# aicodix/modem

Measured on AMD Instinct MI355X. Metric: decoded frames/sec + BER, mode-6 8kHz OFDM, batch 65536, 1/2/4/8 MI355X, higher is better.
Workload: dtype f32

## Files before the change

modem_amd/csrc/k_theilsen.hip:

```cpp
#include "dev_common.h"
#include "kernels.h"

namespace rx {

#define TS_CAP 56
#define TS_OPEN_NEED 30
#define TS_OPEN_MARGIN 6
#define TS_MARGIN 12
#define TS_UNC_STEPS 24
constexpr int TS_QBITS = 22;
constexpr uint32_t TS_QREAL = (1u << TS_QBITS) - 8192u;
constexpr uint32_t TS_QPAD0 = (1u << TS_QBITS) - 4096u;
constexpr uint32_t TS_MQ = 2;
constexpr int TS_MQ1S = (int)((TS_MQ + 1) << 9);
constexpr int TS_LIST = 64;
constexpr int TS_MAX_IT = 48;
constexpr uint32_t TS_SENTINEL = 0x7fffffffu;

constexpr int TS_YS = 68, TS_PS = 76;
#define TS_ROWS_PER_WG 1
#define TS_SYNC() __syncthreads()
struct TsLds {
	float y[8 * TS_YS];
	uint2 sk[8 * TS_PS];
	uint32_t lst[TS_LIST];
};
__device__ __forceinline__ int ts_yaddr(int i) { return (i & 7) * TS_YS + (i >> 3); }
__device__ __forceinline__ int ts_paddr(int p) { return (p & 7) * TS_PS + (p >> 3); }

__device__ __forceinline__ unsigned fkey(float v)
{
	unsigned b = __float_as_uint(v);
	return (b & 0x80000000u) ? ~b : (b | 0x80000000u);
}
__device__ __forceinline__ float fkey_inv(unsigned k)
{
	unsigned b = (k & 0x80000000u) ? (k & 0x7fffffffu) : ~k;
	return __uint_as_float(b);
}
__device__ __forceinline__ float sub_mul_nofma(float y, float s, float x)
{
	#pragma clang fp contract(off)
	float p = s * x;
	return y - p;
}

__device__ __forceinline__ uint32_t med3u(uint32_t a, uint32_t b, uint32_t c)
{
	uint32_t r;
	asm("v_med3_u32 %0, %1, %2, %3" : "=v"(r) : "v"(a), "v"(b), "v"(c));
	return r;
}
template <int CTRL> __device__ __forceinline__ uint32_t dpp_u(uint32_t v)
{
	return (uint32_t)__builtin_amdgcn_mov_dpp((int)v, CTRL, 0xf, 0xf, true);
}
template <int PAT> __device__ __forceinline__ uint32_t swz_u(uint32_t v)
{
	return (uint32_t)__builtin_amdgcn_ds_swizzle((int)v, PAT);
}
constexpr int DPP_XOR1 = 0xB1, DPP_XOR2 = 0x4E, DPP_XOR3 = 0x1B, DPP_HALF_MIRROR = 0x141, DPP_MIRROR = 0x140, DPP_ROR8 = 0x128;
constexpr int SWZ_XOR4 = 0x101F, SWZ_XOR16 = 0x401F, SWZ_XOR31 = 0x7C1F;

struct TsLane {
	uint32_t c1, c2, c4, c8, c16, c32;
	int a63;
	int lane;
};
__device__ __forceinline__ TsLane ts_lane(int lane)
{
	TsLane L;
	L.c1 = (lane & 1) ? ~0u : 0u; L.c2 = (lane & 2) ? ~0u : 0u; L.c4 = (lane & 4) ? ~0u : 0u;
	L.c8 = (lane & 8) ? ~0u : 0u; L.c16 = (lane & 16) ? ~0u : 0u; L.c32 = (lane & 32) ? ~0u : 0u;
	L.a63 = (lane ^ 63) << 2;
	L.lane = lane;
	return L;
}
__device__ __forceinline__ int wave_sum_i(int v)
{
	v += (int)dpp_u<DPP_XOR1>((uint32_t)v);
	v += (int)dpp_u<DPP_XOR2>((uint32_t)v);
	v += (int)dpp_u<DPP_HALF_MIRROR>((uint32_t)v);
	v += (int)dpp_u<DPP_MIRROR>((uint32_t)v);
	return __builtin_amdgcn_readlane(v, 0) + __builtin_amdgcn_readlane(v, 16) + __builtin_amdgcn_readlane(v, 32) + __builtin_amdgcn_readlane(v, 48);
}
__device__ __forceinline__ float ts_uni(float v) { return __uint_as_float(__builtin_amdgcn_readfirstlane(__float_as_uint(v))); }
template <typename Op> __device__ __forceinline__ float wave_reduce_f(float v, Op op)
{
	v = op(v, __uint_as_float(dpp_u<DPP_XOR1>(__float_as_uint(v))));
	v = op(v, __uint_as_float(dpp_u<DPP_XOR2>(__float_as_uint(v))));
	v = op(v, __uint_as_float(dpp_u<DPP_HALF_MIRROR>(__float_as_uint(v))));
	v = op(v, __uint_as_float(dpp_u<DPP_MIRROR>(__float_as_uint(v))));
	const float a = __uint_as_float(__builtin_amdgcn_readlane(__float_as_uint(v), 0)), b = __uint_as_float(__builtin_amdgcn_readlane(__float_as_uint(v), 16));
	const float c = __uint_as_float(__builtin_amdgcn_readlane(__float_as_uint(v), 32)), d = __uint_as_float(__builtin_amdgcn_readlane(__float_as_uint(v), 48));
	return ts_uni(op(op(a, b), op(c, d)));
}

__device__ __forceinline__ void ts_ce(uint32_t &a, uint32_t &b)
{
	const uint32_t lo = a < b ? a : b, hi = a < b ? b : a;
	a = lo; b = hi;
}
template <int D> __device__ __forceinline__ void ts_stage(uint32_t (&k)[8], const TsLane &L)
{
	uint32_t p[8];
	#pragma unroll
	for (int t = 0; t < 8; ++t) {
		if (D == 1) p[t] = dpp_u<DPP_XOR1>(k[t]);
		else if (D == 2) p[t] = dpp_u<DPP_XOR2>(k[t]);
		else if (D == 4) p[t] = swz_u<SWZ_XOR4>(k[t]);
		else if (D == 8) p[t] = dpp_u<DPP_ROR8>(k[t]);
		else p[t] = swz_u<SWZ_XOR16>(k[t]);
	}
	__builtin_amdgcn_sched_barrier(0);
	const uint32_t c = D == 1 ? L.c1 : D == 2 ? L.c2 : D == 4 ? L.c4 : D == 8 ? L.c8 : L.c16;
	#pragma unroll
	for (int t = 0; t < 8; ++t)
		k[t] = med3u(k[t], p[t], c);
	__builtin_amdgcn_sched_barrier(0);
}
template <int M> __device__ __forceinline__ void ts_level(uint32_t (&k)[8], const TsLane &L)
{
	uint32_t p[8];
	#pragma unroll
	for (int t = 0; t < 8; ++t) {
		if (M == 1) p[t] = dpp_u<DPP_XOR1>(k[7 - t]);
		else if (M == 2) p[t] = dpp_u<DPP_XOR3>(k[7 - t]);
		else if (M == 3) p[t] = dpp_u<DPP_HALF_MIRROR>(k[7 - t]);
		else if (M == 4) p[t] = dpp_u<DPP_MIRROR>(k[7 - t]);
		else if (M == 5) p[t] = swz_u<SWZ_XOR31>(k[7 - t]);
		else p[t] = (uint32_t)__builtin_amdgcn_ds_bpermute(L.a63, (int)k[7 - t]);
	}
	__builtin_amdgcn_sched_barrier(0);
	{
		const uint32_t c = M == 1 ? L.c1 : M == 2 ? L.c2 : M == 3 ? L.c4 : M == 4 ? L.c8 : M == 5 ? L.c16 : L.c32;
		#pragma unroll
		for (int t = 0; t < 8; ++t)
			k[t] = med3u(k[t], p[t], c);
	}
	__builtin_amdgcn_sched_barrier(0);
	if (M >= 6) ts_stage<16>(k, L);
	if (M >= 5) ts_stage<8>(k, L);
	if (M >= 4) ts_stage<4>(k, L);
	if (M >= 3) ts_stage<2>(k, L);
	if (M >= 2) ts_stage<1>(k, L);
	ts_ce(k[0], k[4]); ts_ce(k[1], k[5]); ts_ce(k[2], k[6]); ts_ce(k[3], k[7]);
	ts_ce(k[0], k[2]); ts_ce(k[1], k[3]); ts_ce(k[4], k[6]); ts_ce(k[5], k[7]);
	ts_ce(k[0], k[1]); ts_ce(k[2], k[3]); ts_ce(k[4], k[5]); ts_ce(k[6], k[7]);
}
template <int M> __device__ __forceinline__ uint32_t ts_level_count(const uint32_t (&k)[8], const TsLane &L)
{
	uint32_t acc = 0;
	#pragma unroll
	for (int t = 0; t < 8; ++t)
		acc += ((k[t] >> (M + 2)) & 1u) * (256u + t);
	const uint32_t pbase = ((uint32_t)L.lane << 3) & ((16u << (M - 1)) - 1u);
	return (acc >> 8) * pbase + (acc & 255u);
}
constexpr int ts_inv_const()
{
	int c = 0;
	for (int m = 1; m <= 6; ++m) {
		const int k = 8 << m, l = k / 2, runs = 512 / k;
		c += runs * (k * (k - 1) / 2 - l * (l - 1) / 2);
	}
	return c;
}
constexpr int TS_INV_CONST = ts_inv_const();

__device__ __forceinline__ int ts_sort(uint32_t (&k)[8], const TsLane &L, bool counting, int levels)
{
	int share = 0;
	if (counting) {
		uint32_t h = 0;
		#pragma unroll
		for (int t = 0; t < 8; ++t)
			#pragma unroll
			for (int u = t + 1; u < 8; ++u)
				h = __builtin_amdgcn_alignbit(h, k[u] - k[t], 31);
		share = __popc(h);
	}
	ts_ce(k[0], k[1]); ts_ce(k[2], k[3]); ts_ce(k[4], k[5]); ts_ce(k[6], k[7]);
	ts_ce(k[0], k[2]); ts_ce(k[1], k[3]); ts_ce(k[4], k[6]); ts_ce(k[5], k[7]);
	ts_ce(k[1], k[2]); ts_ce(k[5], k[6]);
	ts_ce(k[0], k[4]); ts_ce(k[1], k[5]); ts_ce(k[2], k[6]); ts_ce(k[3], k[7]);
	ts_ce(k[2], k[4]); ts_ce(k[3], k[5]);
	ts_ce(k[1], k[2]); ts_ce(k[3], k[4]); ts_ce(k[5], k[6]);
	ts_level<1>(k, L); if (counting) share -= (int)ts_level_count<1>(k, L);
	ts_level<2>(k, L); if (counting) share -= (int)ts_level_count<2>(k, L);
	ts_level<3>(k, L); if (counting) share -= (int)ts_level_count<3>(k, L);
	ts_level<4>(k, L); if (counting) share -= (int)ts_level_count<4>(k, L);
	if (levels > 4) {
		ts_level<5>(k, L); if (counting) share -= (int)ts_level_count<5>(k, L);
		ts_level<6>(k, L); if (counting) share -= (int)ts_level_count<6>(k, L);
	}
	return share;
}

struct TsQuant { double scale, off; };
__device__ __forceinline__ TsQuant ts_quant(float T, float ymin, float ymax, int n)
{
	const double half = fabs((double)T) * (double)(n / 2 + 1);
	const double lo = (double)ymin - half, span = ((double)ymax + half) - lo;
	float sp = (float)span;
	sp = sp > 1e-30f ? sp : 1e-30f;
	const double scale = (double)(__builtin_amdgcn_rcpf(sp) * ((float)(TS_QREAL - 2u) * (1.f - 9.5367431640625e-7f)));
	TsQuant q;
	q.scale = scale;
	q.off = -lo * scale;
	return q;
}
__device__ __forceinline__ void ts_keys_run(uint32_t (&k)[8], const float (&yv)[8], int idx0, int n, float T, const TsQuant &q)
{
	const double tds = (double)T * q.scale;
	double c = fma(-tds, (double)(idx0 - n / 2), q.off);
	#pragma unroll
	for (int t = 0; t < 8; ++t) {
		const uint32_t qv = (uint32_t)fma((double)yv[t], q.scale, c);
		const int idx = idx0 + t;
		const uint32_t pad = TS_QPAD0 + 8u * (uint32_t)(idx - n + 1);
		k[t] = ((idx < n ? qv : pad) << 9) | (uint32_t)idx;
		c -= tds;
	}
}
__device__ __forceinline__ uint32_t ts_key(float y, int idx, int n, float T, const TsQuant &q)
{
	const double c = fma(-(double)T * q.scale, (double)(idx - n / 2), q.off);
	const uint32_t qv = (uint32_t)fma((double)y, q.scale, c);
	const uint32_t pad = TS_QPAD0 + 8u * (uint32_t)(idx - n + 1);
	return ((idx < n ? qv : pad) << 9) | (uint32_t)idx;
}

__device__ __forceinline__ float ts_pair_slope(const TsLds &s, int a, int b)
{
	const int i = a < b ? a : b, j = a < b ? b : a;
	return (s.y[ts_yaddr(j)] - s.y[ts_yaddr(i)]) / (float)(j - i);
}

__device__ __noinline__ float ts_slow_select(TsLds &s, int n, int lane, int target)
{
	uint32_t prefix = 0, mask = 0;
	int rank = target;
	uint32_t *hist = (uint32_t *)s.sk;
	for (int shift = 24; shift >= 0; shift -= 8) {
		for (int b = lane; b < 256; b += 64)
			hist[b] = 0;
		TS_SYNC();
		for (int d = 1; d < n; ++d) {
			const float fd = (float)d;
			for (int i = lane; i < n - d; i += 64) {
				const unsigned key = fkey((s.y[ts_yaddr(i + d)] - s.y[ts_yaddr(i)]) / fd);
				if ((key & mask) == prefix)
					atomicAdd(&hist[(key >> shift) & 255u], 1u);
			}
		}
		TS_SYNC();
		const uint32_t h0 = hist[4 * lane], h1 = hist[4 * lane + 1], h2 = hist[4 * lane + 2], h3 = hist[4 * lane + 3];
		const int mine = (int)(h0 + h1 + h2 + h3);
		int incl = mine;
		#pragma unroll
		for (int o = 1; o < 64; o <<= 1) {
			const int v = __shfl_up(incl, o);
			if (lane >= o)
				incl += v;
		}
		const int excl = incl - mine;
		const bool here = rank >= excl && rank < incl;
		int bin = 0, rr = 0;
		if (here) {
			rr = rank - excl;
			bin = 4 * lane;
			if (rr >= (int)h0) { rr -= h0; ++bin; if (rr >= (int)h1) { rr -= h1; ++bin; if (rr >= (int)h2) { rr -= h2; ++bin; } } }
		}
		const unsigned long long m = __builtin_amdgcn_ballot_w64(here);
		const int src = m ? __builtin_ctzll(m) : 0;
		bin = __builtin_amdgcn_readlane(bin, src);
		rank = __builtin_amdgcn_readlane(rr, src);
		prefix |= (uint32_t)bin << shift;
		mask |= 255u << shift;
		TS_SYNC();
	}
	return fkey_inv(prefix);
}

__device__ __forceinline__ uint32_t ts_sort_lanes(uint32_t v, const TsLane &L)
{
	v = med3u(v, dpp_u<DPP_XOR1>(v), L.c1);
	v = med3u(v, dpp_u<DPP_XOR3>(v), L.c2); v = med3u(v, dpp_u<DPP_XOR1>(v), L.c1);
	v = med3u(v, dpp_u<DPP_HALF_MIRROR>(v), L.c4); v = med3u(v, dpp_u<DPP_XOR2>(v), L.c2); v = med3u(v, dpp_u<DPP_XOR1>(v), L.c1);
	v = med3u(v, dpp_u<DPP_MIRROR>(v), L.c8); v = med3u(v, swz_u<SWZ_XOR4>(v), L.c4); v = med3u(v, dpp_u<DPP_XOR2>(v), L.c2);
	v = med3u(v, dpp_u<DPP_XOR1>(v), L.c1);
	v = med3u(v, swz_u<SWZ_XOR31>(v), L.c16); v = med3u(v, dpp_u<DPP_ROR8>(v), L.c8); v = med3u(v, swz_u<SWZ_XOR4>(v), L.c4);
	v = med3u(v, dpp_u<DPP_XOR2>(v), L.c2); v = med3u(v, dpp_u<DPP_XOR1>(v), L.c1);
	v = med3u(v, (uint32_t)__builtin_amdgcn_ds_bpermute(L.a63, (int)v), L.c32); v = med3u(v, swz_u<SWZ_XOR16>(v), L.c16);
	v = med3u(v, dpp_u<DPP_ROR8>(v), L.c8); v = med3u(v, swz_u<SWZ_XOR4>(v), L.c4); v = med3u(v, dpp_u<DPP_XOR2>(v), L.c2);
	v = med3u(v, dpp_u<DPP_XOR1>(v), L.c1);
	return v;
}
__device__ __forceinline__ uint32_t wave_max_u(uint32_t v)
{
	uint32_t o;
	o = dpp_u<DPP_XOR1>(v); v = v > o ? v : o;
	o = dpp_u<DPP_XOR2>(v); v = v > o ? v : o;
	o = dpp_u<DPP_HALF_MIRROR>(v); v = v > o ? v : o;
	o = dpp_u<DPP_MIRROR>(v); v = v > o ? v : o;
	const uint32_t a = __builtin_amdgcn_readlane(v, 0), b = __builtin_amdgcn_readlane(v, 16), c = __builtin_amdgcn_readlane(v, 32), d = __builtin_amdgcn_readlane(v, 48);
	const uint32_t ab = a > b ? a : b, cd = c > d ? c : d;
	return ab > cd ? ab : cd;
}

__device__ __forceinline__ float2 theil_sen_wave(TsLds &s, int n, int lane)
{
	const TsLane L = ts_lane(lane);
	const int count = n * (n - 1) / 2, target = count / 2, xoff = n / 2;
	float slope = 0.f;
	uint32_t k[8];
	auto load_y = [&](float (&yv)[8]) {
		#pragma unroll
		for (int t = 0; t < 8; ++t)
			yv[t] = 8 * lane + t < n ? s.y[t * TS_YS + lane] : 0.f;
	};
	if (lane < TS_PS - 64) {
		#pragma unroll
		for (int t = 0; t < 8; ++t)
			s.sk[t * TS_PS + 64 + lane] = make_uint2(TS_SENTINEL, TS_SENTINEL);
	}
	bool sorted_z = false;
	if (count > 0) {
		float ymin = 3.0e38f, ymax = -3.0e38f, sy = 0.f, sxy = 0.f;
		{
		float yv[8];
		load_y(yv);
		#pragma unroll
		for (int t = 0; t < 8; ++t) {
			const int i = 8 * lane + t;
			if (i < n) {
				ymin = fminf(ymin, yv[t]); ymax = fmaxf(ymax, yv[t]);
				sy += yv[t]; sxy += yv[t] * (float)(i - xoff);
			}
		}
		}
		ymin = wave_reduce_f(ymin, [](float a, float b) { return fminf(a, b); });
		ymax = wave_reduce_f(ymax, [](float a, float b) { return fmaxf(a, b); });
		sy = wave_reduce_f(sy, [](float a, float b) { return a + b; });
		sxy = wave_reduce_f(sxy, [](float a, float b) { return a + b; });
		bool done = false, slow = false;
		if (ymin == ymax)
			done = true;
		else if (!(ymax - ymin < 3.0e38f)) {
			slow = true;
		}
		float Ta = 0.f, Tb = 0.f, T = 0.f;
		int ca = 0, cb = count;
		bool hasA = false, hasB = false;
		TsQuant qs = {0.0, 0.0};
		const unsigned long long real_lanes = n >= 512 ? ~0ull : (1ull << ((n + 7) >> 3)) - 1ull;
		float Tp = 0.f, irho = 0.f;
		int cp = 0, it = 0, c_at_T = 0;
		bool hasP = false, open_end = false, open_failed = false;
		float To_open = 0.f;
		if (!done && !slow) {
			{
				const float fn = (float)n, sx = fn * (fn - 1.f) * 0.5f - fn * (float)xoff;
				const float sxx = (fn - 1.f) * fn * (2.f * fn - 1.f) * (1.f / 6.f) - 2.f * (float)xoff * (fn * (fn - 1.f) * 0.5f) + fn * (float)xoff * (float)xoff;
				const float rn = __builtin_amdgcn_rcpf(fn);
				T = (sxy - sx * sy * rn) * __builtin_amdgcn_rcpf(sxx - sx * sx * rn);
				if (!(fabsf(T) < 1.0e30f))
					T = 0.f;
				T = ts_uni(T);
			}
		}
		for (;;) {
		if (!done && !slow) {
			for (;; ++it) {
				if (it >= TS_MAX_IT) { slow = true; break; }
				qs = ts_quant(T, ymin, ymax, n);
				{
					float yv[8];
					load_y(yv);
					ts_keys_run(k, yv, 8 * lane, n, T, qs);
				}
				const int share = ts_sort(k, L, true, 6);
				int c_lt = TS_INV_CONST + wave_sum_i(share), c_le;
				TS_SYNC();
				#pragma unroll
				for (int t = 0; t < 8; ++t)
					s.sk[t * TS_PS + lane].x = k[t];
				TS_SYNC();
				{
					int dmin = (int)(s.sk[lane + 1].x - k[7]);
					#pragma unroll
					for (int t = 0; t < 7; ++t) {
						const int d = (int)(k[t + 1] - k[t]);
						dmin = d < dmin ? d : dmin;
					}
					int dlt = 0, dle = 0;
					if (__builtin_amdgcn_ballot_w64(dmin < TS_MQ1S)) {
						for (int kk = 1;; ++kk) {
							if (kk > TS_UNC_STEPS) { slow = true; break; }
							uint32_t h = 0;
							#pragma unroll
							for (int t = 0; t < 8; ++t)
								h = __builtin_amdgcn_alignbit(h, s.sk[((t + kk) & 7) * TS_PS + lane + ((t + kk) >> 3)].x - k[t] - (uint32_t)TS_MQ1S, 31);
							if (!__builtin_amdgcn_ballot_w64(h != 0))
								break;
							while (__builtin_amdgcn_ballot_w64(h != 0)) {
								if (h != 0) {
									const int bit = 31 - __clz(h), p = 8 * lane + 7 - bit;
									h &= ~(1u << bit);
									const int a = (int)(s.sk[ts_paddr(p)].x & 511u), b = (int)(s.sk[ts_paddr(p + kk)].x & 511u);
									const int counted = a > b;
									const float sl = ts_pair_slope(s, a, b);
									dlt += (sl < T) - counted;
									dle += (sl <= T) - counted;
								}
							}
						}
						if (slow)
							break;
						dlt = wave_sum_i(dlt);
						dle = wave_sum_i(dle);
					}
					c_le = c_lt + dle;
					c_lt += dlt;
				}
				sorted_z = true;
				c_at_T = c_lt;
				if (c_lt <= target && target < c_le) { slope = T; done = true; break; }
				if (c_lt <= target) { Ta = T; ca = c_lt; hasA = true; }
				else { Tb = T; cb = c_lt; hasB = true; }
				if (hasA && hasB) {
					if (cb - ca <= TS_CAP)
						break;
					if (fkey(Tb) - fkey(Ta) <= 1u) { slope = Ta; done = true; break; }
				}
				if (it == 0) {
					const uint32_t q1 = s.sk[ts_paddr(n / 4)].x >> 9, q3 = s.sk[ts_paddr((3 * n) / 4)].x >> 9;
					const float iqr = (float)(q3 > q1 ? q3 - q1 : 1u) * __builtin_amdgcn_rcpf((float)qs.scale);
					const float fn = (float)n;
					irho = ts_uni(iqr * (2.f * 1.7724539f * 6.f / 1.349f) * __builtin_amdgcn_rcpf(fn * (fn * fn - 1.f)));
				}
				if (hasP && c_lt != cp && T != Tp)
					irho = ts_uni((T - Tp) * __builtin_amdgcn_rcpf((float)(c_lt - cp)));
				{
					const bool below = c_lt <= target;
					const int need = below ? target - c_lt + 1 : c_lt - target;
					if (!open_failed && irho > 0.f && need <= TS_OPEN_NEED) {
						const float w = (float)(need + TS_OPEN_MARGIN) * irho * 1.25f;
						To_open = ts_uni(below ? T + w : T - w);
						if (fabsf(To_open) < 1.0e30f && To_open != T && (below ? (!hasB || To_open < Tb) : (!hasA || To_open > Ta))) {
							open_end = true;
							break;
						}
					}
				}
				int goal;
				if (it == 0 && !open_failed) goal = target;
				else if (!hasA) goal = target - TS_MARGIN;
				else if (!hasB) goal = target + TS_MARGIN;
				else goal = (target - ca > cb - target) ? target - TS_MARGIN : target + TS_MARGIN;
				float Tn = T;
				bool ok = false;
				if (irho > 0.f && it < 10) {
					Tn = T + ((float)(goal - c_lt) + 0.5f) * irho;
					ok = fabsf(Tn) < 1.0e30f && Tn != T && (!hasA || Tn > Ta) && (!hasB || Tn < Tb);
				}
				if (!ok) {
					const uint32_t ka = hasA ? fkey(Ta) : fkey(-1.0e30f), kb = hasB ? fkey(Tb) : fkey(1.0e30f);
					uint32_t km = ka + (kb - ka) / 2u;
					if (km == ka)
						km = kb;
					Tn = fkey_inv(km);
					if (Tn == T) { slow = true; break; }
				}
				Tp = T; cp = c_lt; hasP = true;
				T = ts_uni(Tn);
			}
		}
		if (!done && !slow) {
			const bool t_is_a = open_end ? c_at_T <= target : T == Ta;
			const float To = open_end ? To_open : (t_is_a ? Tb : Ta);
			const float La = t_is_a ? T : To, Lb = t_is_a ? To : T;
			const TsQuant qo = ts_quant(To, ymin, ymax, n);
			#pragma unroll
			for (int t = 0; t < 8; ++t) {
				const int i = (int)(k[t] & 511u);
				s.sk[t * TS_PS + lane].y = ts_key(i < n ? s.y[ts_yaddr(i)] : 0.f, i, n, To, qo);
			}
			const float wq = fabsf(Lb - La) * (float)qs.scale * (float)(n - 1) * 1.0001f + 4.f;
			const int ws = wq < 4.0e6f ? (int)(((uint32_t)wq << 9) | 511u) : 0x7fffffff;
			TS_SYNC();
			int nc = 0;
			for (int kk = 1;; ++kk) {
				if (kk > 8 * (TS_PS - 64)) {
					slow = true; break;
				}
				uint32_t h = 0;
				int gmin = 0x7fffffff;
				#pragma unroll
				for (int t = 0; t < 8; ++t) {
					const uint2 o = s.sk[((t + kk) & 7) * TS_PS + lane + ((t + kk) >> 3)];
					const int x2 = (int)o.x - ((int)k[t] + TS_MQ1S);
					const int x1 = (int)o.y - ((int)s.sk[t * TS_PS + lane].y + TS_MQ1S);
					const int x2r = o.x < (TS_QPAD0 << 9) ? x2 : 0x7fffffff;
					gmin = x2r < gmin ? x2r : gmin;
					h = __builtin_amdgcn_alignbit(h, (uint32_t)(x1 | x2), 31);
				}
				unsigned long long hm = __builtin_amdgcn_ballot_w64(h != 0);
				while (hm) {
					const bool mine = h != 0;
					const int slot = nc + (int)__builtin_amdgcn_mbcnt_hi((unsigned)(hm >> 32), __builtin_amdgcn_mbcnt_lo((unsigned)hm, 0));
					if (mine) {
						const int bit = 31 - __clz(h), p = 8 * lane + 7 - bit;
						h &= ~(1u << bit);
						if (slot < TS_LIST)
							s.lst[slot] = (uint32_t)p | ((uint32_t)(p + kk) << 16);
					}
					nc += __popcll(hm);
					hm = __builtin_amdgcn_ballot_w64(h != 0);
				}
				if (!(__builtin_amdgcn_ballot_w64(gmin <= ws) & real_lanes))
					break;
			}
			TS_SYNC();
			bool retry = false;
			if (nc > TS_LIST) {
				if (open_end)
					retry = true;
				else {
					slow = true;
				}
			}
			if (!slow && !retry) {
				bool in = false;
				uint32_t key = 0xffffffffu;
				if (lane < nc) {
					const uint32_t e = s.lst[lane];
					const float sl = ts_pair_slope(s, (int)(s.sk[ts_paddr(e & 0xffffu)].x & 511u), (int)(s.sk[ts_paddr(e >> 16)].x & 511u));
					in = sl >= La && sl < Lb;
					if (in)
						key = fkey(sl);
				}
				const int found = __popcll(__builtin_amdgcn_ballot_w64(in));
				const int idx = t_is_a ? target - c_at_T : found - (c_at_T - target);
				if (open_end) {
					if (idx < 0 || idx >= found)
						retry = true;
				} else if (found != cb - ca) {
					slow = true;
				}
				if (!slow && !retry) {
					key = ts_sort_lanes(key, L);
					slope = fkey_inv(__builtin_amdgcn_readlane(key, idx));
				}
			}
			if (retry) {
				open_failed = true;
				open_end = false;
				Tp = T; cp = c_at_T; hasP = true;
				T = To;
				++it;
				continue;
			}
		}
		break;
		}
		if (slow) {
			slope = ts_slow_select(s, n, lane, target);
			sorted_z = false;
		}
	}
	float yint = 0.f;
	bool have = false;
	if (sorted_z) {
		uint32_t bk[8];
		#pragma unroll
		for (int t = 0; t < 8; ++t) {
			const int i = (int)(k[t] & 511u);
			bk[t] = i < n ? fkey(sub_mul_nofma(s.y[ts_yaddr(i)], slope, (float)(i - xoff))) : 0xffffffffu;
		}
		TS_SYNC();
		if (lane == (n / 2) >> 3) {
			#pragma unroll
			for (int t = 0; t < 8; ++t)
				if (t == ((n / 2) & 7))
					s.lst[0] = bk[t];
		}
		TS_SYNC();
		uint32_t cand = s.lst[0];
		for (int round = 0; round < 6 && !have; ++round) {
			int both = 0;
			#pragma unroll
			for (int t = 0; t < 8; ++t)
				both += (int)(bk[t] < cand) + ((int)(bk[t] <= cand) << 16);
			both = wave_sum_i(both);
			const int lt = both & 0xffff, le = both >> 16;
			if (lt <= n / 2 && n / 2 < le) {
				have = true;
			} else if (lt > n / 2) {
				uint32_t m = 0;
				#pragma unroll
				for (int t = 0; t < 8; ++t)
					m = (bk[t] < cand && bk[t] > m) ? bk[t] : m;
				cand = wave_max_u(m);
			} else {
				uint32_t m = 0;
				#pragma unroll
				for (int t = 0; t < 8; ++t)
					m = (bk[t] > cand && ~bk[t] > m) ? ~bk[t] : m;
				cand = ~wave_max_u(m);
			}
		}
		yint = fkey_inv(cand);
	}
	if (!have) {
		float yv[8];
		load_y(yv);
		#pragma unroll
		for (int t = 0; t < 8; ++t) {
			const int i = 8 * lane + t;
			k[t] = i < n ? fkey(sub_mul_nofma(yv[t], slope, (float)(i - xoff))) : 0xffffffffu;
		}
		ts_sort(k, L, false, 6);
		TS_SYNC();
		#pragma unroll
		for (int t = 0; t < 8; ++t)
			s.sk[t * TS_PS + lane].x = k[t];
		TS_SYNC();
		yint = n > 0 ? fkey_inv(s.sk[ts_paddr(n / 2)].x) : 0.f;
	}
	return make_float2(slope, yint);
}

#define TS_OWN_ATAN 1
__device__ __forceinline__ float ts_phase(cf d, int mod_bits)
{
	const float lim = mod_bits == 3 ? 0.42f : 1.005f;
	if (!TS_OWN_ATAN || !(d.re > 0.f) || !(fabsf(d.im) <= lim * d.re))
		return atan2f(d.im, d.re);
	const float r = __builtin_amdgcn_rcpf(d.re);
	float t = d.im * r;
	t = fmaf(fmaf(-d.re, t, d.im), r, t);
	const float z = t * t;
	float p;
	if (mod_bits == 3) {
		p = -5.951132927e-02f;
		p = fmaf(p, z, 1.054106507e-01f);
		p = fmaf(p, z, -1.423576012e-01f);
		p = fmaf(p, z, 1.999798680e-01f);
		p = fmaf(p, z, -3.333330347e-01f);
		p = fmaf(p, z, 9.999999993e-01f);
	} else {
		p = -1.718391760e-03f;
		p = fmaf(p, z, 1.059115275e-02f);
		p = fmaf(p, z, -3.059610274e-02f);
		p = fmaf(p, z, 5.738879400e-02f);
		p = fmaf(p, z, -8.370542419e-02f);
		p = fmaf(p, z, 1.094069024e-01f);
		p = fmaf(p, z, -1.426187097e-01f);
		p = fmaf(p, z, 1.999827962e-01f);
		p = fmaf(p, z, -3.333328490e-01f);
		p = fmaf(p, z, 9.999999978e-01f);
	}
	return p * t;
}

__device__ __forceinline__ void ts_row(TsLds &s, int f, int j, int lane, const ModeDesc &md, cf *__restrict__ cons_all,
	const cf *__restrict__ carr_all, float *__restrict__ slope_all, float *__restrict__ yint_all)
{
	const int cols = md.cols;
	cf *row = cons_all + (size_t)f * CONS_MAX + (size_t)j * cols;
	const cf *cr = carr_all ? carr_all + (size_t)f * CARR_MAX + (size_t)j * cols : nullptr;
	cf pt[8], pv[8];
	#pragma unroll
	for (int q = 0; q < 8; ++q) {
		const int i = lane + 64 * q;
		if (i < cols) {
			if (cr) {
				pt[q] = cr[cols + i];
				pv[q] = cr[i];
			} else
				pt[q] = row[i];
		}
	}
	#pragma unroll
	for (int q = 0; q < 8; ++q) {
		const int i = lane + 64 * q;
		if (i < cols) {
			cf c = pt[q];
			if (cr) {
				c = demod_or_erase(pt[q], pv[q]);
				row[i] = c;
			}
			cf d = cmul(c, cconj(md.mod_bits == 3 ? psk8_hard_map(c) : psk4_hard_map(c)));
			s.y[ts_yaddr(i)] = ts_phase(d, md.mod_bits);
		}
	}
	TS_SYNC();
	const float2 sy = theil_sen_wave(s, cols, lane);
	if (lane == 0) {
		slope_all[(size_t)f * ROWS_MAX + j] = sy.x;
		yint_all[(size_t)f * ROWS_MAX + j] = sy.y;
	}
}

#define TS_MORE_WAVES_N 20480
#define TS_MORE_OCC 5
constexpr int TS_ROWS_DIRECT = 50, TS_MORE_WAVES = TS_MORE_WAVES_N;
__global__ __launch_bounds__(64 * TS_ROWS_PER_WG, 5) void k_theil_sen(const SyncState *__restrict__ st_all, cf *__restrict__ cons_all,
	const cf *__restrict__ carr_all, float *__restrict__ slope_all, float *__restrict__ yint_all, int n_frames, int *__restrict__ chunk_flags)
{
	const int unit = (int)blockIdx.x * TS_ROWS_PER_WG + ((int)threadIdx.x >> 6);
	const int f = __builtin_amdgcn_readfirstlane(unit / TS_ROWS_DIRECT), j = __builtin_amdgcn_readfirstlane(unit % TS_ROWS_DIRECT), lane = threadIdx.x & 63;
	if (f >= n_frames || !st_all[f].okay)
		return;
	const ModeDesc md = mode_desc(st_all[f].oper_mode);
	if (j == 0 && lane == 0 && md.rows > TS_ROWS_DIRECT)
		atomicMax(chunk_flags, md.rows);
	if (j >= md.rows)
		return;
	__shared__ TsLds s_all[TS_ROWS_PER_WG];
	ts_row(s_all[threadIdx.x >> 6], f, j, lane, md, cons_all, carr_all, slope_all, yint_all);
}
__global__ __launch_bounds__(64, TS_MORE_OCC) void k_theil_sen_more(const SyncState *__restrict__ st_all, cf *__restrict__ cons_all,
	const cf *__restrict__ carr_all, float *__restrict__ slope_all, float *__restrict__ yint_all, int n_frames, const int *__restrict__ chunk_flags)
{
	const int more = chunk_flags[0] - TS_ROWS_DIRECT;
	if (more <= 0)
		return;
	const int lane = threadIdx.x, units = n_frames * more;
	__shared__ TsLds s;
	for (int u = (int)blockIdx.x; u < units; u += TS_MORE_WAVES) {
		const int f = u / more, j = TS_ROWS_DIRECT + u % more;
		if (!st_all[f].okay)
			continue;
		const ModeDesc md = mode_desc(st_all[f].oper_mode);
		if (j >= md.rows)
			continue;
		__syncthreads();
		ts_row(s, f, j, lane, md, cons_all, carr_all, slope_all, yint_all);
	}
}
__global__ __launch_bounds__(64 * TS_ROWS_PER_WG, 5) void k_theil_sen_raw(int cols, int rows, const float *__restrict__ y, float *__restrict__ slope_all,
	float *__restrict__ yint_all)
{
	const int r = __builtin_amdgcn_readfirstlane((int)blockIdx.x * TS_ROWS_PER_WG + ((int)threadIdx.x >> 6)), lane = threadIdx.x & 63;
	if (r >= rows)
		return;
	__shared__ TsLds s_all[TS_ROWS_PER_WG];
	TsLds &s = s_all[threadIdx.x >> 6];
	for (int i = lane; i < cols; i += 64)
		s.y[ts_yaddr(i)] = y[(size_t)r * cols + i];
	TS_SYNC();
	const float2 sy = theil_sen_wave(s, cols, lane);
	if (lane == 0) { slope_all[r] = sy.x; yint_all[r] = sy.y; }
}

void launch_theil_sen(hipStream_t s, int n, const SyncState *st, cf *cons, const cf *carr, float *slope, float *yint, int *chunk_flags)
{
	hipLaunchKernelGGL(k_theil_sen, dim3((n * TS_ROWS_DIRECT + TS_ROWS_PER_WG - 1) / TS_ROWS_PER_WG), dim3(64 * TS_ROWS_PER_WG), 0, s, st, cons, carr,
		slope, yint, n, chunk_flags);
	hipLaunchKernelGGL(k_theil_sen_more, dim3(TS_MORE_WAVES), dim3(64), 0, s, st, cons, carr, slope, yint, n,
		chunk_flags);
}
void launch_theil_sen_raw(hipStream_t s, int rows, int cols, const float *y, float *slope, float *yint)
{
	hipLaunchKernelGGL(k_theil_sen_raw, dim3((rows + TS_ROWS_PER_WG - 1) / TS_ROWS_PER_WG), dim3(64 * TS_ROWS_PER_WG), 0, s, cols, rows, y, slope, yint);
}

}
```

Before: 1.855 million.

## Drop second key set in Theil-Sen bracketing; use f32 quantization and paired reductions

Result: faster. 1.985 million, median of 6 (+7.0%).

```diff
diff --git a/modem_amd/csrc/k_theilsen.hip b/modem_amd/csrc/k_theilsen.hip
--- a/modem_amd/csrc/k_theilsen.hip
+++ b/modem_amd/csrc/k_theilsen.hip
@@ -11,8 +11,10 @@
 constexpr int TS_QBITS = 22;
 constexpr uint32_t TS_QREAL = (1u << TS_QBITS) - 8192u;
 constexpr uint32_t TS_QPAD0 = (1u << TS_QBITS) - 4096u;
-constexpr uint32_t TS_MQ = 2;
+constexpr uint32_t TS_MQ = 3;
 constexpr int TS_MQ1S = (int)((TS_MQ + 1) << 9);
+constexpr int TS_FLIP_C = 512 * 3 + 511;
+static_assert(TS_MQ >= 3, "the list's test covers the uncertain pairs up to dq = 3 only: see TS_FLIP_C");
 constexpr int TS_LIST = 64;
 constexpr int TS_MAX_IT = 48;
 constexpr uint32_t TS_SENTINEL = 0x7fffffffu;
@@ -22,7 +24,7 @@
 #define TS_SYNC() __syncthreads()
 struct TsLds {
 	float y[8 * TS_YS];
-	uint2 sk[8 * TS_PS];
+	uint32_t sk[8 * TS_PS];
 	uint32_t lst[TS_LIST];
 };
 __device__ __forceinline__ int ts_yaddr(int i) { return (i & 7) * TS_YS + (i >> 3); }
@@ -95,6 +97,29 @@
 	const float c = __uint_as_float(__builtin_amdgcn_readlane(__float_as_uint(v), 32)), d = __uint_as_float(__builtin_amdgcn_readlane(__float_as_uint(v), 48));
 	return ts_uni(op(op(a, b), op(c, d)));
 }
+
+constexpr int DPP_ROR4 = 0x124;
+template <typename Op> __device__ __forceinline__ void wave_reduce_f2(float &a, float &b, bool odd, Op op)
+{
+	a = op(a, __uint_as_float(dpp_u<DPP_XOR1>(__float_as_uint(a))));
+	b = op(b, __uint_as_float(dpp_u<DPP_XOR1>(__float_as_uint(b))));
+	float v = odd ? b : a;
+	v = op(v, __uint_as_float(dpp_u<DPP_XOR2>(__float_as_uint(v))));
+	v = op(v, __uint_as_float(dpp_u<DPP_ROR4>(__float_as_uint(v))));
+	v = op(v, __uint_as_float(dpp_u<DPP_ROR8>(__float_as_uint(v))));
+	const uint32_t u = __float_as_uint(v);
+	auto rl = [&](int l) { return __uint_as_float(__builtin_amdgcn_readlane(u, l)); };
+	a = ts_uni(op(op(rl(0), rl(16)), op(rl(32), rl(48))));
+	b = ts_uni(op(op(rl(1), rl(17)), op(rl(33), rl(49))));
+}
+struct TsStat {
+	float ymin = 3.0e38f, ymax = -3.0e38f, sy = 0.f, sxy = 0.f;
+	__device__ __forceinline__ void add(float y, int i, int xoff)
+	{
+		ymin = fminf(ymin, y); ymax = fmaxf(ymax, y);
+		sy += y; sxy = fmaf(y, (float)(i - xoff), sxy);
+	}
+};
 
 __device__ __forceinline__ void ts_ce(uint32_t &a, uint32_t &b)
 {
@@ -148,14 +173,21 @@
 	ts_ce(k[0], k[2]); ts_ce(k[1], k[3]); ts_ce(k[4], k[6]); ts_ce(k[5], k[7]);
 	ts_ce(k[0], k[1]); ts_ce(k[2], k[3]); ts_ce(k[4], k[5]); ts_ce(k[6], k[7]);
 }
+template <int M> __device__ __forceinline__ uint32_t ts_level_bits(const uint32_t (&k)[8], int t0)
+{
+	constexpr uint32_t s = (M + 2) >> 3, bb = (M + 2) & 7;
+	uint32_t p = __builtin_amdgcn_perm(k[t0 + 1], k[t0], 0x0c0c0000u | ((4u + s) << 8) | s);
+	p = __builtin_amdgcn_perm(k[t0 + 2], p, 0x0c000100u | ((4u + s) << 16));
+	p = __builtin_amdgcn_perm(k[t0 + 3], p, 0x00020100u | ((4u + s) << 24));
+	return p & (0x01010101u << bb);
+}
 template <int M> __device__ __forceinline__ uint32_t ts_level_count(const uint32_t (&k)[8], const TsLane &L)
 {
-	uint32_t acc = 0;
-	#pragma unroll
-	for (int t = 0; t < 8; ++t)
-		acc += ((k[t] >> (M + 2)) & 1u) * (256u + t);
+	const uint32_t a = ts_level_bits<M>(k, 0), b = ts_level_bits<M>(k, 4);
+	const uint32_t cnt = __builtin_amdgcn_udot4(a, 0x01010101u, __builtin_amdgcn_udot4(b, 0x01010101u, 0u, false), false);
+	const uint32_t tw = __builtin_amdgcn_udot4(a, 0x03020100u, __builtin_amdgcn_udot4(b, 0x07060504u, 0u, false), false);
 	const uint32_t pbase = ((uint32_t)L.lane << 3) & ((16u << (M - 1)) - 1u);
-	return (acc >> 8) * pbase + (acc & 255u);
+	return (__umul24(cnt, pbase) + tw) >> ((M + 2) & 7);
 }
 constexpr int ts_inv_const()
 {
@@ -197,38 +229,29 @@
 	return share;
 }
 
-struct TsQuant { double scale, off; };
+struct TsQuant { float scale, tds, off; };
 __device__ __forceinline__ TsQuant ts_quant(float T, float ymin, float ymax, int n)
 {
-	const double half = fabs((double)T) * (double)(n / 2 + 1);
-	const double lo = (double)ymin - half, span = ((double)ymax + half) - lo;
-	float sp = (float)span;
+	const float half = fabsf(T) * (float)(n / 2 + 1);
+	float sp = fmaf(2.f, half, ymax - ymin);
 	sp = sp > 1e-30f ? sp : 1e-30f;
-	const double scale = (double)(__builtin_amdgcn_rcpf(sp) * ((float)(TS_QREAL - 2u) * (1.f - 9.5367431640625e-7f)));
 	TsQuant q;
-	q.scale = scale;
-	q.off = -lo * scale;
+	q.scale = ts_uni(__builtin_amdgcn_rcpf(sp) * ((float)(TS_QREAL - 2u) * (1.f - 9.5367431640625e-7f)));
+	q.tds = ts_uni(T * q.scale);
+	q.off = ts_uni(half * q.scale);
 	return q;
 }
-__device__ __forceinline__ void ts_keys_run(uint32_t (&k)[8], const float (&yv)[8], int idx0, int n, float T, const TsQuant &q)
-{
-	const double tds = (double)T * q.scale;
-	double c = fma(-tds, (double)(idx0 - n / 2), q.off);
+__device__ __forceinline__ void ts_keys_run(uint32_t (&k)[8], const float (&yv)[8], int idx0, int n, float ymin, const TsQuant &q)
+{
+	const float c0 = fmaf(-q.tds, (float)(idx0 - n / 2), q.off);
 	#pragma unroll
 	for (int t = 0; t < 8; ++t) {
-		const uint32_t qv = (uint32_t)fma((double)yv[t], q.scale, c);
+		const float c = t ? fmaf(-(float)t, q.tds, c0) : c0;
+		const uint32_t qv = (uint32_t)fmaf(yv[t] - ymin, q.scale, c);
 		const int idx = idx0 + t;
 		const uint32_t pad = TS_QPAD0 + 8u * (uint32_t)(idx - n + 1);
 		k[t] = ((idx < n ? qv : pad) << 9) | (uint32_t)idx;
-		c -= tds;
-	}
-}
-__device__ __forceinline__ uint32_t ts_key(float y, int idx, int n, float T, const TsQuant &q)
-{
-	const double c = fma(-(double)T * q.scale, (double)(idx - n / 2), q.off);
-	const uint32_t qv = (uint32_t)fma((double)y, q.scale, c);
-	const uint32_t pad = TS_QPAD0 + 8u * (uint32_t)(idx - n + 1);
-	return ((idx < n ? qv : pad) << 9) | (uint32_t)idx;
+	}
 }
 
 __device__ __forceinline__ float ts_pair_slope(const TsLds &s, int a, int b)
@@ -309,7 +332,7 @@
 	return ab > cd ? ab : cd;
 }
 
-__device__ __forceinline__ float2 theil_sen_wave(TsLds &s, int n, int lane)
+__device__ __forceinline__ float2 theil_sen_wave(TsLds &s, int n, int lane, const TsStat &st)
 {
 	const TsLane L = ts_lane(lane);
 	const int count = n * (n - 1) / 2, target = count / 2, xoff = n / 2;
@@ -323,27 +346,14 @@
 	if (lane < TS_PS - 64) {
 		#pragma unroll
 		for (int t = 0; t < 8; ++t)
-			s.sk[t * TS_PS + 64 + lane] = make_uint2(TS_SENTINEL, TS_SENTINEL);
+			s.sk[t * TS_PS + 64 + lane] = TS_SENTINEL;
 	}
 	bool sorted_z = false;
 	if (count > 0) {
-		float ymin = 3.0e38f, ymax = -3.0e38f, sy = 0.f, sxy = 0.f;
-		{
-		float yv[8];
-		load_y(yv);
-		#pragma unroll
-		for (int t = 0; t < 8; ++t) {
-			const int i = 8 * lane + t;
-			if (i < n) {
-				ymin = fminf(ymin, yv[t]); ymax = fmaxf(ymax, yv[t]);
-				sy += yv[t]; sxy += yv[t] * (float)(i - xoff);
-			}
-		}
-		}
-		ymin = wave_reduce_f(ymin, [](float a, float b) { return fminf(a, b); });
-		ymax = wave_reduce_f(ymax, [](float a, float b) { return fmaxf(a, b); });
-		sy = wave_reduce_f(sy, [](float a, float b) { return a + b; });
-		sxy = wave_reduce_f(sxy, [](float a, float b) { return a + b; });
+		float ymin = st.ymin, nmax = -st.ymax, sy = st.sy, sxy = st.sxy;
+		wave_reduce_f2(ymin, nmax, lane & 1, [](float a, float b) { return fminf(a, b); });
+		wave_reduce_f2(sy, sxy, lane & 1, [](float a, float b) { return a + b; });
+		const float ymax = -nmax;
 		bool done = false, slow = false;
 		if (ymin == ymax)
 			done = true;
@@ -353,7 +363,7 @@
 		float Ta = 0.f, Tb = 0.f, T = 0.f;
 		int ca = 0, cb = count;
 		bool hasA = false, hasB = false;
-		TsQuant qs = {0.0, 0.0};
+		TsQuant qs = {0.f, 0.f, 0.f};
 		const unsigned long long real_lanes = n >= 512 ? ~0ull : (1ull << ((n + 7) >> 3)) - 1ull;
 		float Tp = 0.f, irho = 0.f;
 		int cp = 0, it = 0, c_at_T = 0;
@@ -378,17 +388,17 @@
 				{
 					float yv[8];
 					load_y(yv);
-					ts_keys_run(k, yv, 8 * lane, n, T, qs);
+					ts_keys_run(k, yv, 8 * lane, n, ymin, qs);
 				}
 				const int share = ts_sort(k, L, true, 6);
 				int c_lt = TS_INV_CONST + wave_sum_i(share), c_le;
 				TS_SYNC();
 				#pragma unroll
 				for (int t = 0; t < 8; ++t)
-					s.sk[t * TS_PS + lane].x = k[t];
+					s.sk[t * TS_PS + lane] = k[t];
 				TS_SYNC();
 				{
-					int dmin = (int)(s.sk[lane + 1].x - k[7]);
+					int dmin = (int)(s.sk[lane + 1] - k[7]);
 					#pragma unroll
 					for (int t = 0; t < 7; ++t) {
 						const int d = (int)(k[t + 1] - k[t]);
@@ -401,14 +411,14 @@
 							uint32_t h = 0;
 							#pragma unroll
 							for (int t = 0; t < 8; ++t)
-								h = __builtin_amdgcn_alignbit(h, s.sk[((t + kk) & 7) * TS_PS + lane + ((t + kk) >> 3)].x - k[t] - (uint32_t)TS_MQ1S, 31);
+								h = __builtin_amdgcn_alignbit(h, s.sk[((t + kk) & 7) * TS_PS + lane + ((t + kk) >> 3)] - k[t] - (uint32_t)TS_MQ1S, 31);
 							if (!__builtin_amdgcn_ballot_w64(h != 0))
 								break;
 							while (__builtin_amdgcn_ballot_w64(h != 0)) {
 								if (h != 0) {
 									const int bit = 31 - __clz(h), p = 8 * lane + 7 - bit;
 									h &= ~(1u << bit);
-									const int a = (int)(s.sk[ts_paddr(p)].x & 511u), b = (int)(s.sk[ts_paddr(p + kk)].x & 511u);
+									const int a = (int)(s.sk[ts_paddr(p)] & 511u), b = (int)(s.sk[ts_paddr(p + kk)] & 511u);
 									const int counted = a > b;
 									const float sl = ts_pair_slope(s, a, b);
 									dlt += (sl < T) - counted;
@@ -435,8 +445,8 @@
 					if (fkey(Tb) - fkey(Ta) <= 1u) { slope = Ta; done = true; break; }
 				}
 				if (it == 0) {
-					const uint32_t q1 = s.sk[ts_paddr(n / 4)].x >> 9, q3 = s.sk[ts_paddr((3 * n) / 4)].x >> 9;
-					const float iqr = (float)(q3 > q1 ? q3 - q1 : 1u) * __builtin_amdgcn_rcpf((float)qs.scale);
+					const uint32_t q1 = s.sk[ts_paddr(n / 4)] >> 9, q3 = s.sk[ts_paddr((3 * n) / 4)] >> 9;
+					const float iqr = (float)(q3 > q1 ? q3 - q1 : 1u) * __builtin_amdgcn_rcpf(qs.scale);
 					const float fn = (float)n;
 					irho = ts_uni(iqr * (2.f * 1.7724539f * 6.f / 1.349f) * __builtin_amdgcn_rcpf(fn * (fn * fn - 1.f)));
 				}
@@ -481,17 +491,17 @@
 			const bool t_is_a = open_end ? c_at_T <= target : T == Ta;
 			const float To = open_end ? To_open : (t_is_a ? Tb : Ta);
 			const float La = t_is_a ? T : To, Lb = t_is_a ? To : T;
-			const TsQuant qo = ts_quant(To, ymin, ymax, n);
+			const float w512 = fabsf(Lb - La) * qs.scale * (512.f * 1.000001f);
+			const bool too_wide = !(w512 < 2.0e6f);
+			const int wi = too_wide ? 0 : (int)w512 + 1, wis = __builtin_amdgcn_readfirstlane(t_is_a ? wi : -wi);
+			const float wq = fabsf(Lb - La) * qs.scale * (float)(n - 1) * 1.0001f + 4.f;
+			const int ws = too_wide ? 0 : (int)(((uint32_t)wq << 9) | 511u);
+			int nb[8];
 			#pragma unroll
-			for (int t = 0; t < 8; ++t) {
-				const int i = (int)(k[t] & 511u);
-				s.sk[t * TS_PS + lane].y = ts_key(i < n ? s.y[ts_yaddr(i)] : 0.f, i, n, To, qo);
-			}
-			const float wq = fabsf(Lb - La) * (float)qs.scale * (float)(n - 1) * 1.0001f + 4.f;
-			const int ws = wq < 4.0e6f ? (int)(((uint32_t)wq << 9) | 511u) : 0x7fffffff;
-			TS_SYNC();
-			int nc = 0;
-			for (int kk = 1;; ++kk) {
+			for (int t = 0; t < 8; ++t)
+				nb[t] = (TS_FLIP_C + 1) - __mul24(wis, (int)(k[t] & 511u));
+			int nc = too_wide ? TS_LIST + 1 : 0;
+			for (int kk = 1; !too_wide; ++kk) {
 				if (kk > 8 * (TS_PS - 64)) {
 					slow = true; break;
 				}
@@ -499,12 +509,11 @@
 				int gmin = 0x7fffffff;
 				#pragma unroll
 				for (int t = 0; t < 8; ++t) {
-					const uint2 o = s.sk[((t + kk) & 7) * TS_PS + lane + ((t + kk) >> 3)];
-					const int x2 = (int)o.x - ((int)k[t] + TS_MQ1S);
-					const int x1 = (int)o.y - ((int)s.sk[t * TS_PS + lane].y + TS_MQ1S);
-					const int x2r = o.x < (TS_QPAD0 << 9) ? x2 : 0x7fffffff;
-					gmin = x2r < gmin ? x2r : gmin;
-					h = __builtin_amdgcn_alignbit(h, (uint32_t)(x1 | x2), 31);
+					const uint32_t o = s.sk[((t + kk) & 7) * TS_PS + lane + ((t + kk) >> 3)];
+					const int dk = o < (TS_QPAD0 << 9) ? (int)(o - k[t]) : 0x7fffffff;
+					const int thr = max(__mul24(wis, (int)(o & 511u)) + nb[t], TS_FLIP_C + 1);
+					gmin = dk < gmin ? dk : gmin;
+					h = __builtin_amdgcn_alignbit(h, (uint32_t)(dk - thr), 31);
 				}
 				unsigned long long hm = __builtin_amdgcn_ballot_w64(h != 0);
 				while (hm) {
@@ -519,7 +528,7 @@
 					nc += __popcll(hm);
 					hm = __builtin_amdgcn_ballot_w64(h != 0);
 				}
-				if (!(__builtin_amdgcn_ballot_w64(gmin <= ws) & real_lanes))
+				if (!(__builtin_amdgcn_ballot_w64(gmin - TS_MQ1S <= ws) & real_lanes))
 					break;
 			}
 			TS_SYNC();
@@ -536,7 +545,7 @@
 				uint32_t key = 0xffffffffu;
 				if (lane < nc) {
 					const uint32_t e = s.lst[lane];
-					const float sl = ts_pair_slope(s, (int)(s.sk[ts_paddr(e & 0xffffu)].x & 511u), (int)(s.sk[ts_paddr(e >> 16)].x & 511u));
+					const float sl = ts_pair_slope(s, (int)(s.sk[ts_paddr(e & 0xffffu)] & 511u), (int)(s.sk[ts_paddr(e >> 16)] & 511u));
 					in = sl >= La && sl < Lb;
 					if (in)
 						key = fkey(sl);
@@ -625,9 +634,9 @@
 		TS_SYNC();
 		#pragma unroll
 		for (int t = 0; t < 8; ++t)
-			s.sk[t * TS_PS + lane].x = k[t];
+			s.sk[t * TS_PS + lane] = k[t];
 		TS_SYNC();
-		yint = n > 0 ? fkey_inv(s.sk[ts_paddr(n / 2)].x) : 0.f;
+		yint = n > 0 ? fkey_inv(s.sk[ts_paddr(n / 2)]) : 0.f;
 	}
 	return make_float2(slope, yint);
 }
@@ -683,6 +692,7 @@
 				pt[q] = row[i];
 		}
 	}
+	TsStat st;
 	#pragma unroll
 	for (int q = 0; q < 8; ++q) {
 		const int i = lane + 64 * q;
@@ -693,11 +703,13 @@
 				row[i] = c;
 			}
 			cf d = cmul(c, cconj(md.mod_bits == 3 ? psk8_hard_map(c) : psk4_hard_map(c)));
-			s.y[ts_yaddr(i)] = ts_phase(d, md.mod_bits);
+			const float ph = ts_phase(d, md.mod_bits);
+			s.y[ts_yaddr(i)] = ph;
+			st.add(ph, i, cols / 2);
 		}
 	}
 	TS_SYNC();
-	const float2 sy = theil_sen_wave(s, cols, lane);
+	const float2 sy = theil_sen_wave(s, cols, lane, st);
 	if (lane == 0) {
 		slope_all[(size_t)f * ROWS_MAX + j] = sy.x;
 		yint_all[(size_t)f * ROWS_MAX + j] = sy.y;
@@ -749,10 +761,14 @@
 		return;
 	__shared__ TsLds s_all[TS_ROWS_PER_WG];
 	TsLds &s = s_all[threadIdx.x >> 6];
-	for (int i = lane; i < cols; i += 64)
-		s.y[ts_yaddr(i)] = y[(size_t)r * cols + i];
+	TsStat st;
+	for (int i = lane; i < cols; i += 64) {
+		const float v = y[(size_t)r * cols + i];
+		s.y[ts_yaddr(i)] = v;
+		st.add(v, i, cols / 2);
+	}
 	TS_SYNC();
-	const float2 sy = theil_sen_wave(s, cols, lane);
+	const float2 sy = theil_sen_wave(s, cols, lane, st);
 	if (lane == 0) { slope_all[r] = sy.x; yint_all[r] = sy.y; }
 }
 
```
